# c-zhou/oatk

Hardware: AMD Instinct MI355X
Metric: HiFi Gbases/s through syncasm (syncmer+syncerr) at k=1001 s=31 (higher is better)
Workload: dtype u64

## Files before the change

### oatk_amd/csrc/kmer_hash.hpp

```cpp
#pragma once
#include "common.hpp"
#include "count.hpp"

namespace oatk {

struct KmerHashArgs {
    const uint8_t *hoco_s;
    const uint64_t *off;
    uint64_t sid0;
    const uint64_t *raw_lo;
    const uint64_t *raw_smer;
    const uint32_t *raw_mpos;
    const uint32_t *shard_cnt;
    uint32_t region_cap;
    const uint64_t *scm_off;
    uint64_t hash_mask;
    uint64_t *pos_hash, *pos_lo, *pos_smer;
    uint32_t *pos_mpos;
    uint64_t *key_hash;
    uint32_t *iota;
    uint4 *slot_rec;
    int K;
};

#define KMH_REC 16
#define KMH_WG_WAVES 4
#define KMH_WG_REC (KMH_REC * KMH_WG_WAVES)
#define KMH_WPL 8

__device__ __forceinline__ uint32_t kmh_rev_in_bytes(uint32_t x)
{
    x = ((x >> 2) & 0x33333333u) | ((x & 0x33333333u) << 2);
    return ((x >> 4) & 0x0F0F0F0Fu) | ((x & 0x0F0F0F0Fu) << 4);
}

__host__ __device__ inline int kmh_lds_stride(int K)
{
    const int nbytes = (K - 1) / 4 + 1;
    return ((nbytes + 7) >> 3) | 1;
}
__host__ __device__ inline size_t kmh_lds_bytes(int K) { return (size_t) KMH_WG_REC * kmh_lds_stride(K) * 8; }

#ifndef OATK_KMH_WAVES
#define OATK_KMH_WAVES 8
#endif
__global__ __launch_bounds__(KMH_WG_WAVES * 64, OATK_KMH_WAVES) void kmer_hash_kernel(KmerHashArgs a)
{
    extern __shared__ uint64_t kmix[];
    const uint32_t lane = threadIdx.x & 63u, q = lane & 3u;
    const uint32_t wave = __builtin_amdgcn_readfirstlane(threadIdx.x >> 6);
    const uint32_t rr = wave * (uint32_t) KMH_REC + (lane >> 2);
    const uint32_t base = blockIdx.x * (uint32_t) KMH_WG_REC;
    uint32_t cnt = a.shard_cnt[blockIdx.y];
    cnt = cnt < a.region_cap? cnt : a.region_cap;
    if (base >= cnt) return;
    const size_t src = (size_t) blockIdx.y * a.region_cap + base;
    const int K = a.K;
    const int nbytes = (K - 1) / 4 + 1, nfull = nbytes >> 3, nrem = nbytes & 7, NW = nfull + (nrem? 1 : 0);
    const int stride = kmh_lds_stride(K);
    const uint32_t nrec = cnt - base < (uint32_t) KMH_WG_REC? cnt - base : (uint32_t) KMH_WG_REC;
    if (rr < nrec) {
        const uint32_t mp = a.raw_mpos[src + rr];
        const uint64_t lo = a.raw_lo[src + rr];
        const uint32_t rev = mp & 1u, pos = mp >> 1;
        const int64_t hsw = (int64_t) (a.off[(lo >> 32) - a.sid0] >> 4);
        const uint32_t *hs32 = (const uint32_t *) a.hoco_s;
        uint64_t *out = &kmix[rr * (uint32_t) stride];
        const int per = (NW + 3) >> 2;
        for (int w0 = (int) q * per; w0 < (int) (q + 1) * per && w0 < NW; w0 += KMH_WPL) {
            const int nwd = (int) (q + 1) * per - w0 < KMH_WPL? (int) (q + 1) * per - w0 : KMH_WPL;
            const int n = w0 + nwd > NW? NW - w0 : nwd;
            const int32_t t_lo = rev? (int32_t) pos + K - 32 * (w0 + n) : (int32_t) pos + 32 * w0;
            const int32_t wi = t_lo >> 4;
            const uint32_t sh = ((uint32_t) t_lo & 15u) * 2u;
            uint32_t asc[2 * KMH_WPL + 1];
            const int64_t gbase = hsw + wi;
            if (n == KMH_WPL && gbase >= 0) {
                struct __attribute__((packed, aligned(4))) W4 { uint32_t a, b, c, e; };
                const W4 *src = (const W4 *) (hs32 + gbase);
                const W4 v0 = src[0], v1 = src[1], v2 = src[2], v3 = src[3];
                const uint32_t v4 = hs32[gbase + 16];
                const uint32_t raw[17] = {v0.a, v0.b, v0.c, v0.e, v1.a, v1.b, v1.c, v1.e, v2.a, v2.b, v2.c, v2.e, v3.a, v3.b, v3.c, v3.e, v4};
#pragma unroll
                for (int i = 0; i < 17; ++i) asc[i] = __builtin_bswap32(raw[i]);
            } else {
#pragma unroll
                for (int i = 0; i < 2 * KMH_WPL + 1; ++i) {
                    int64_t gi = gbase + i;
                    gi = gi < 0? 0 : gi;
                    asc[i] = i < 2 * n + 1? __builtin_bswap32(hs32[gi]) : 0u;
                }
            }
#pragma unroll
            for (int c = 0; c < KMH_WPL; ++c) {
                if (c >= n) break;
                const uint32_t x0 = asc[2 * c], x1 = asc[2 * c + 1], x2 = asc[2 * c + 2];
                const uint32_t hi = (uint32_t) (((uint64_t) x0 << 32 | x1) >> (32u - sh));
                const uint32_t lo = (uint32_t) (((uint64_t) x1 << 32 | x2) >> (32u - sh));
                const int j = rev? n - 1 - c : c;
                const int wd = w0 + j;
                int nb = K - 32 * wd;
                nb = nb > 32? 32 : nb;
                uint64_t word;
                if (rev) {
                    uint64_t V = (uint64_t) hi << 32 | lo;
                    if (nb < 32) V &= ~0ULL >> (64 - 2 * nb);
                    const uint64_t R = revcomp32(V);
                    word = nb < 32? bswap64(R & (~0ULL << (64 - 2 * nb)))
                                  : ~((uint64_t) kmh_rev_in_bytes(hi) << 32 | kmh_rev_in_bytes(lo));
                } else {
                    uint64_t V = (uint64_t) hi << 32 | lo;
                    if (nb < 32) V &= ~0ULL << (64 - 2 * nb);
                    word = bswap64(V);
                }
                out[wd] = wd < nfull? murmur_mix_word(word) : word;
            }
        }
    }
    const uint32_t mine = lane < nrec? lane : nrec - 1;
    uint64_t my_lo = 0;
    if (wave == 0) my_lo = a.raw_lo[src + mine];
    __syncthreads();
    if (wave != 0) return;
    const uint64_t my_sm = a.raw_smer[src + mine];
    const uint32_t my_mp = a.raw_mpos[src + mine];
    const uint64_t my_off = a.scm_off[(my_lo >> 32) - a.sid0];
    const uint32_t my_hsw = (uint32_t) (a.off[(my_lo >> 32) - a.sid0] >> 4);
    const uint64_t *km = &kmix[mine * (uint32_t) stride];
    uint64_t h = OATK_MURMUR_SEED ^ ((uint64_t) (uint32_t) nbytes * OATK_MURMUR_M);
    for (int wd = 0; wd < nfull; ++wd) h = (h ^ km[wd]) * OATK_MURMUR_M;
    if (nrem) h = (h ^ km[nfull]) * OATK_MURMUR_M;
    h ^= h >> 47; h *= OATK_MURMUR_M; h ^= h >> 47;
    if (lane < nrec) {
        const uint64_t my_p = my_off + ((uint32_t) my_lo >> 1);
        a.pos_hash[my_p] = h, a.key_hash[my_p] = h & a.hash_mask;
        a.pos_lo[my_p] = my_lo, a.pos_smer[my_p] = my_sm, a.pos_mpos[my_p] = my_mp, a.iota[my_p] = (uint32_t) my_p;
        a.slot_rec[2 * (size_t) my_p] = make_uint4((uint32_t) my_lo, (uint32_t) (my_lo >> 32), (uint32_t) my_sm, (uint32_t) (my_sm >> 32));
        a.slot_rec[2 * (size_t) my_p + 1] = make_uint4(my_mp, my_hsw, 0u, 0u);
    }
}

}
```

Measured before the change: 436.6.

## Sort k-mer records by strand within workgroup to remove strand divergence

Each wave ballots the strand bit of its 64 records and writes a forward-first permutation into a small LDS order array. Records are then assigned so forward and reverse records mostly land in separate waves, and a templated prepare routine runs the strand-specific path without divergence. The full-width fast path also drops per-word tail masking and handles only the last word with a precomputed mask. This costs extra LDS, a ballot/shuffle prologue, and a larger code footprint from instantiating both template variants.

```diff
diff --git a/oatk_amd/csrc/kmer_hash.hpp b/oatk_amd/csrc/kmer_hash.hpp
--- a/oatk_amd/csrc/kmer_hash.hpp
+++ b/oatk_amd/csrc/kmer_hash.hpp
@@ -39,7 +39,76 @@
     const int nbytes = (K - 1) / 4 + 1;
     return ((nbytes + 7) >> 3) | 1;
 }
-__host__ __device__ inline size_t kmh_lds_bytes(int K) { return (size_t) KMH_WG_REC * kmh_lds_stride(K) * 8; }
+__host__ __device__ inline size_t kmh_lds_bytes(int K) { return (size_t) KMH_WG_REC * kmh_lds_stride(K) * 8 + KMH_WG_REC; }
+
+template <bool REV>
+__device__ __forceinline__ void kmh_prepare(const uint32_t *hs32, int64_t hsw, uint32_t pos, int K, int NW, int nfull, uint32_t q, uint64_t *out)
+{
+    const int per = (NW + 3) >> 2;
+    for (int w0 = (int) q * per; w0 < (int) (q + 1) * per && w0 < NW; w0 += KMH_WPL) {
+        const int nwd = (int) (q + 1) * per - w0 < KMH_WPL? (int) (q + 1) * per - w0 : KMH_WPL;
+        const int n = w0 + nwd > NW? NW - w0 : nwd;
+        const int32_t t_lo = REV? (int32_t) pos + K - 32 * (w0 + n) : (int32_t) pos + 32 * w0;
+        const int32_t wi = t_lo >> 4;
+        const uint32_t sh = ((uint32_t) t_lo & 15u) * 2u;
+        uint32_t asc[2 * KMH_WPL + 1];
+        const int64_t gbase = hsw + wi;
+        if (n == KMH_WPL && gbase >= 0) {
+            struct __attribute__((packed, aligned(4))) W4 { uint32_t a, b, c, e; };
+            const W4 *src = (const W4 *) (hs32 + gbase);
+            const W4 v0 = src[0], v1 = src[1], v2 = src[2], v3 = src[3];
+            const uint32_t v4 = hs32[gbase + 16];
+            const uint32_t raw[17] = {v0.a, v0.b, v0.c, v0.e, v1.a, v1.b, v1.c, v1.e, v2.a, v2.b, v2.c, v2.e, v3.a, v3.b, v3.c, v3.e, v4};
+#pragma unroll
+            for (int i = 0; i < 17; ++i) asc[i] = __builtin_bswap32(raw[i]);
+            const int wl = w0 + KMH_WPL - 1;
+            int nbl = K - 32 * wl;
+            nbl = nbl > 32? 32 : nbl;
+            const uint64_t keep = bswap64(~0ULL << (64 - 2 * nbl));
+#pragma unroll
+            for (int c = 0; c < KMH_WPL; ++c) {
+                const uint32_t x0 = asc[2 * c], x1 = asc[2 * c + 1], x2 = asc[2 * c + 2];
+                const uint32_t hi = (uint32_t) (((uint64_t) x0 << 32 | x1) >> (32u - sh));
+                const uint32_t lo = (uint32_t) (((uint64_t) x1 << 32 | x2) >> (32u - sh));
+                const uint64_t word = REV? ~((uint64_t) kmh_rev_in_bytes(hi) << 32 | kmh_rev_in_bytes(lo)) : bswap64((uint64_t) hi << 32 | lo);
+                const int j = REV? KMH_WPL - 1 - c : c;
+                if (j == KMH_WPL - 1) out[wl] = wl < nfull? murmur_mix_word(word & keep) : word & keep;
+                else out[w0 + j] = murmur_mix_word(word);
+            }
+            continue;
+        }
+#pragma unroll
+        for (int i = 0; i < 2 * KMH_WPL + 1; ++i) {
+            int64_t gi = gbase + i;
+            gi = gi < 0? 0 : gi;
+            asc[i] = i < 2 * n + 1? __builtin_bswap32(hs32[gi]) : 0u;
+        }
+#pragma unroll
+        for (int c = 0; c < KMH_WPL; ++c) {
+            if (c >= n) break;
+            const uint32_t x0 = asc[2 * c], x1 = asc[2 * c + 1], x2 = asc[2 * c + 2];
+            const uint32_t hi = (uint32_t) (((uint64_t) x0 << 32 | x1) >> (32u - sh));
+            const uint32_t lo = (uint32_t) (((uint64_t) x1 << 32 | x2) >> (32u - sh));
+            const int j = REV? n - 1 - c : c;
+            const int wd = w0 + j;
+            int nb = K - 32 * wd;
+            nb = nb > 32? 32 : nb;
+            uint64_t word;
+            if (REV) {
+                uint64_t V = (uint64_t) hi << 32 | lo;
+                if (nb < 32) V &= ~0ULL >> (64 - 2 * nb);
+                const uint64_t R = revcomp32(V);
+                word = nb < 32? bswap64(R & (~0ULL << (64 - 2 * nb)))
+                              : ~((uint64_t) kmh_rev_in_bytes(hi) << 32 | kmh_rev_in_bytes(lo));
+            } else {
+                uint64_t V = (uint64_t) hi << 32 | lo;
+                if (nb < 32) V &= ~0ULL << (64 - 2 * nb);
+                word = bswap64(V);
+            }
+            out[wd] = wd < nfull? murmur_mix_word(word) : word;
+        }
+    }
+}
 
 #ifndef OATK_KMH_WAVES
 #define OATK_KMH_WAVES 8
@@ -49,7 +118,7 @@
     extern __shared__ uint64_t kmix[];
     const uint32_t lane = threadIdx.x & 63u, q = lane & 3u;
     const uint32_t wave = __builtin_amdgcn_readfirstlane(threadIdx.x >> 6);
-    const uint32_t rr = wave * (uint32_t) KMH_REC + (lane >> 2);
+    const uint32_t e = wave * (uint32_t) KMH_REC + (lane >> 2);
     const uint32_t base = blockIdx.x * (uint32_t) KMH_WG_REC;
     uint32_t cnt = a.shard_cnt[blockIdx.y];
     cnt = cnt < a.region_cap? cnt : a.region_cap;
@@ -59,71 +128,40 @@
     const int nbytes = (K - 1) / 4 + 1, nfull = nbytes >> 3, nrem = nbytes & 7, NW = nfull + (nrem? 1 : 0);
     const int stride = kmh_lds_stride(K);
     const uint32_t nrec = cnt - base < (uint32_t) KMH_WG_REC? cnt - base : (uint32_t) KMH_WG_REC;
-    if (rr < nrec) {
-        const uint32_t mp = a.raw_mpos[src + rr];
+    const uint32_t mine = lane < nrec? lane : nrec - 1;
+    const uint32_t mp_l = a.raw_mpos[src + mine];
+    const uint64_t fwd_m = __ballot(lane < nrec && !(mp_l & 1u)), rev_m = __ballot(lane < nrec && (mp_l & 1u));
+    const uint32_t nf = (uint32_t) __builtin_popcountll(fwd_m);
+    uint8_t *order = (uint8_t *) (kmix + (size_t) KMH_WG_REC * (uint32_t) stride);
+    {
+        const uint32_t at = (mp_l & 1u)? nf + __builtin_amdgcn_mbcnt_hi((uint32_t) (rev_m >> 32), __builtin_amdgcn_mbcnt_lo((uint32_t) rev_m, 0u))
+                                       : __builtin_amdgcn_mbcnt_hi((uint32_t) (fwd_m >> 32), __builtin_amdgcn_mbcnt_lo((uint32_t) fwd_m, 0u));
+        if (lane < nrec && (at >> 4) == wave) order[at] = (uint8_t) lane;
+        __builtin_amdgcn_fence(__ATOMIC_RELEASE, "wavefront");
+        __builtin_amdgcn_wave_barrier();
+        __builtin_amdgcn_fence(__ATOMIC_ACQUIRE, "wavefront");
+    }
+    const uint32_t rr = e < nrec? order[e] : 0u;
+    const uint32_t pos = (uint32_t) __shfl((int) mp_l, (int) rr) >> 1;
+    if (e < nrec) {
         const uint64_t lo = a.raw_lo[src + rr];
-        const uint32_t rev = mp & 1u, pos = mp >> 1;
         const int64_t hsw = (int64_t) (a.off[(lo >> 32) - a.sid0] >> 4);
         const uint32_t *hs32 = (const uint32_t *) a.hoco_s;
         uint64_t *out = &kmix[rr * (uint32_t) stride];
-        const int per = (NW + 3) >> 2;
-        for (int w0 = (int) q * per; w0 < (int) (q + 1) * per && w0 < NW; w0 += KMH_WPL) {
-            const int nwd = (int) (q + 1) * per - w0 < KMH_WPL? (int) (q + 1) * per - w0 : KMH_WPL;
-            const int n = w0 + nwd > NW? NW - w0 : nwd;
-            const int32_t t_lo = rev? (int32_t) pos + K - 32 * (w0 + n) : (int32_t) pos + 32 * w0;
-            const int32_t wi = t_lo >> 4;
-            const uint32_t sh = ((uint32_t) t_lo & 15u) * 2u;
-            uint32_t asc[2 * KMH_WPL + 1];
-            const int64_t gbase = hsw + wi;
-            if (n == KMH_WPL && gbase >= 0) {
-                struct __attribute__((packed, aligned(4))) W4 { uint32_t a, b, c, e; };
-                const W4 *src = (const W4 *) (hs32 + gbase);
-                const W4 v0 = src[0], v1 = src[1], v2 = src[2], v3 = src[3];
-                const uint32_t v4 = hs32[gbase + 16];
-                const uint32_t raw[17] = {v0.a, v0.b, v0.c, v0.e, v1.a, v1.b, v1.c, v1.e, v2.a, v2.b, v2.c, v2.e, v3.a, v3.b, v3.c, v3.e, v4};
-#pragma unroll
-                for (int i = 0; i < 17; ++i) asc[i] = __builtin_bswap32(raw[i]);
-            } else {
-#pragma unroll
-                for (int i = 0; i < 2 * KMH_WPL + 1; ++i) {
-                    int64_t gi = gbase + i;
-                    gi = gi < 0? 0 : gi;
-                    asc[i] = i < 2 * n + 1? __builtin_bswap32(hs32[gi]) : 0u;
-                }
-            }
-#pragma unroll
-            for (int c = 0; c < KMH_WPL; ++c) {
-                if (c >= n) break;
-                const uint32_t x0 = asc[2 * c], x1 = asc[2 * c + 1], x2 = asc[2 * c + 2];
-                const uint32_t hi = (uint32_t) (((uint64_t) x0 << 32 | x1) >> (32u - sh));
-                const uint32_t lo = (uint32_t) (((uint64_t) x1 << 32 | x2) >> (32u - sh));
-                const int j = rev? n - 1 - c : c;
-                const int wd = w0 + j;
-                int nb = K - 32 * wd;
-                nb = nb > 32? 32 : nb;
-                uint64_t word;
-                if (rev) {
-                    uint64_t V = (uint64_t) hi << 32 | lo;
-                    if (nb < 32) V &= ~0ULL >> (64 - 2 * nb);
-                    const uint64_t R = revcomp32(V);
-                    word = nb < 32? bswap64(R & (~0ULL << (64 - 2 * nb)))
-                                  : ~((uint64_t) kmh_rev_in_bytes(hi) << 32 | kmh_rev_in_bytes(lo));
-                } else {
-                    uint64_t V = (uint64_t) hi << 32 | lo;
-                    if (nb < 32) V &= ~0ULL << (64 - 2 * nb);
-                    word = bswap64(V);
-                }
-                out[wd] = wd < nfull? murmur_mix_word(word) : word;
-            }
+        const uint32_t e0 = wave * (uint32_t) KMH_REC, e1 = e0 + KMH_REC < nrec? e0 + KMH_REC : nrec;
+        if (e0 < nf) {
+            if (e < nf) kmh_prepare<false>(hs32, hsw, pos, K, NW, nfull, q, out);
+        }
+        if (e1 > nf) {
+            if (e >= nf) kmh_prepare<true>(hs32, hsw, pos, K, NW, nfull, q, out);
         }
     }
-    const uint32_t mine = lane < nrec? lane : nrec - 1;
     uint64_t my_lo = 0;
     if (wave == 0) my_lo = a.raw_lo[src + mine];
     __syncthreads();
     if (wave != 0) return;
     const uint64_t my_sm = a.raw_smer[src + mine];
-    const uint32_t my_mp = a.raw_mpos[src + mine];
+    const uint32_t my_mp = mp_l;
     const uint64_t my_off = a.scm_off[(my_lo >> 32) - a.sid0];
     const uint32_t my_hsw = (uint32_t) (a.off[(my_lo >> 32) - a.sid0] >> 4);
     const uint64_t *km = &kmix[mine * (uint32_t) stride];
```

Result: no change. 434.5 (-0.5%).
